# umr-lops/xsarsea

Hardware: AMD Instinct MI355X
Metric: Mpixels/s wind inversion (CMOD5.N, 20k x 20k sigma0) (higher is better)
Workload: dtype f64; 1 GPU; CMOD5.N mono-VV inversion (the metric's raster), 20000x20000 float32 sigma0/incidence + complex64 ancillary, default LUT 501x499x181 (90319 candidates/pixel), complex64 out, algo=pruned, sigma0 -> dB fused on the device; lines=20000, samples=20000, lines_rank0=20000, parallelism=row tiles x1

## Files before the change

profiles/band_vpipe_isa.py:

```python
#!/usr/bin/env python3
import collections
import os
import re
import subprocess
import sys
import tempfile

HERE = os.path.dirname(os.path.abspath(__file__))
sys.path.insert(0, HERE)
from stage1_isa_breakdown import CSRC, REPO, function_starts

KERNELS = [
    ("k_invert_band mono, table in LDS (the benchmark's)", "13k_invert_bandIffLb0ELb0ELi1ELb1EE"),
    ("k_invert_band mono, table in global memory", "13k_invert_bandIffLb0ELb0ELi1ELb0EE"),
    ("k_invert_band dual-pol, table in LDS", "13k_invert_bandIffLb1ELb0ELi1ELb1EE"),
    ("k_invert_band dual-pol, table in global memory", "13k_invert_bandIffLb1ELb0ELi1ELb0EE"),
    ("k_invert_band2 mono", "14k_invert_band2IffLb0EE"),
    ("k_invert_band2 dual-pol", "14k_invert_band2IffLb1EE"),
    ("k_invert_blocks mono", "15k_invert_blocksIffLb0EE"),
    ("k_invert_blocks dual-pol", "15k_invert_blocksIffLb1EE"),
]
HELPERS = {"vmin", "vmax", "vminf", "vmaxf", "dpp_d", "dpp_f", "seg_min_d", "wave_min_d", "rd_lane_d", "rd_lane_i", "mul24_sv", "wave_max_i",
           "ballot64", "byte_sum4", "ld", "to_db", "log10_fast"}
TAIL_FUNCS = {"wave_tail", "list_append", "mask_mark", "store_pixel", "angle_of_quotient", "hypot_glibc", "search_cr_scan", "search_cr_interval",
              "dsig_cr_at", "nearest_index_tail", "co_encode", "cr_encode", "store_opt"}
PASS_FUNCS = {"co_band_pass", "ld_co"}


def compile_asm(path):
    subprocess.check_call(["/opt/rocm/bin/hipcc", "--offload-arch=gfx950", "-O3", "-std=c++17", "-ffp-contract=off", "-I" + os.path.join(REPO, "include"),
                           "-I" + CSRC, "-DXSW_PAIR=0", "-gline-tables-only", "--cuda-device-only", "-S", os.path.join(CSRC, "xsw_invert_tu.hip"), "-o", path],
                          stderr=subprocess.DEVNULL)
    return open(path).read().split("\n")


def kind_of(op):
    if op.startswith(("global_", "flat_", "buffer_", "scratch_")):
        return "VMEM"
    if op.startswith("ds_"):
        return "LDS"
    if op.startswith(("s_load_", "s_buffer_load_")):
        return "SMEM"
    return "SALU" if op.startswith("s_") else "VALU"


def main():
    if len(sys.argv) > 1:
        text = open(sys.argv[1]).read().split("\n")
    else:
        with tempfile.TemporaryDirectory() as td:
            text = compile_asm(os.path.join(td, "tu.s"))
    files = {}
    for line in text:
        m = re.match(r'\s*\.file\s+(\d+)\s+"([^"]*)"\s+"([^"]*)"', line)
        if m:
            files[int(m.group(1))] = os.path.basename(m.group(3))
    headers = ("xsw_device.hpp", "xsw_band.hpp", "xsw_band2.hpp", "xsw_blocks.hpp", "xsw_codes.hpp")
    fstarts = {f: function_starts(os.path.join(CSRC, f)) for f in headers}
    band_src = open(os.path.join(CSRC, "xsw_band.hpp")).read().split("\n")
    l_passes = next(n for n, l in enumerate(band_src, 1) if "// ---- stage 2: band passes" in l)
    l_pickup = next(n for n, l in enumerate(band_src, 1) if "the workgroup's passes have settled every slot" in l)

    def phase_of(fname, line, prev):
        if fname not in fstarts:
# ... 89 lines not shown
```

xsarsea_amd/_build.py:

```python
import os
import shutil
import subprocess

HERE = os.path.dirname(os.path.abspath(__file__))
REPO = os.path.dirname(HERE)
CSRC = os.path.join(HERE, "csrc")
SRC = os.path.join(CSRC, "xsw.hip")
SRC_TU = os.path.join(CSRC, "xsw_invert_tu.hip")
SRC_GRAD = os.path.join(CSRC, "xsw_gradients.hip")
SRC_STREAKS = os.path.join(CSRC, "xsw_streaks.hip")
SRC_ANCILLARY = os.path.join(CSRC, "xsw_ancillary.hip")
SRC_CELLS = os.path.join(CSRC, "xsw_cells.hip")
SRC_CALIBRATE = os.path.join(CSRC, "xsw_calibrate.hip")
SRC_LANDMASK = os.path.join(CSRC, "xsw_landmask.hip")
DEPS = [os.path.join(CSRC, f) for f in sorted(os.listdir(CSRC)) if f.endswith((".hip", ".hpp"))] + [os.path.join(REPO, "include", "xsw.h")]
LIB = os.environ.get("XSW_LIB") or os.path.join(HERE, "libxsw.so")
OBJDIR = os.path.join(REPO, "build", "obj")
ARCH = "gfx950"


def hipcc():
    for cand in (shutil.which("hipcc"), "/opt/rocm/bin/hipcc"):
        if cand and os.path.exists(cand):
            return cand
    raise RuntimeError("hipcc not found: libxsw.so cannot be built")


def needs_build():
    if not os.path.exists(LIB):
        return True
    t = os.path.getmtime(LIB)
    return any(os.path.getmtime(d) > t for d in DEPS)


def build(force=False, verbose=False):
    if not force and not needs_build():
        return LIB
    cc = hipcc()
    extra = os.environ.get("XSW_EXTRA_FLAGS", "").split()
    tag = os.path.basename(LIB).replace(".", "_")
    os.makedirs(OBJDIR, exist_ok=True)
    common = [cc, f"--offload-arch={ARCH}", "-O3", "-std=c++17", "-ffp-contract=off", "-fPIC",
              "-I" + os.path.join(REPO, "include"), "-I" + CSRC] + extra
    jobs = [(SRC, os.path.join(OBJDIR, f"{tag}_main.o"), [])]
    jobs += [(SRC_TU, os.path.join(OBJDIR, f"{tag}_pair{k}.o"), [f"-DXSW_PAIR={k}"]) for k in range(4)]
    jobs += [(SRC_GRAD, os.path.join(OBJDIR, f"{tag}_gradients.o"), [])]
    jobs += [(SRC_STREAKS, os.path.join(OBJDIR, f"{tag}_streaks.o"), [])]
    jobs += [(SRC_ANCILLARY, os.path.join(OBJDIR, f"{tag}_ancillary.o"), [])]
    jobs += [(SRC_CELLS, os.path.join(OBJDIR, f"{tag}_cells.o"), [])]
    jobs += [(SRC_CALIBRATE, os.path.join(OBJDIR, f"{tag}_calibrate.o"), [])]
    jobs += [(SRC_LANDMASK, os.path.join(OBJDIR, f"{tag}_landmask.o"), [])]
    procs = []
    for src, obj, defs in jobs:
        cmd = common + defs + ["-c", src, "-o", obj]
        if verbose:
            print(" ".join(cmd))
        procs.append((cmd, subprocess.Popen(cmd)))
    failed = [cmd for cmd, p in procs if p.wait() != 0]
    if failed:
        raise subprocess.CalledProcessError(1, failed[0])
    link = [cc, f"--offload-arch={ARCH}", "-shared", "-fPIC", "-o", LIB] + [obj for _, obj, _ in jobs] + ["-Wl,-rpath,/opt/rocm/lib"]
    if verbose:
        print(" ".join(link))
    subprocess.check_call(link)
    return LIB


def _code_objects(lib, td):
    llvm = "/opt/rocm/lib/llvm/bin"
    fat = os.path.join(td, "fat.bin")
    subprocess.check_call([f"{llvm}/llvm-objcopy", "--dump-section", f".hip_fatbin={fat}", lib, os.path.join(td, "unused.so")])
    with open(fat, "rb") as f:
        blob = f.read()
    magic = b"__CLANG_OFFLOAD_BUNDLE__"
    starts = [m for m in range(len(blob)) if blob.startswith(magic, m)] if blob.count(magic) < 64 else []
    out = []
    for k, st in enumerate(starts):
        piece, co = os.path.join(td, f"bundle{k}.bin"), os.path.join(td, f"dev{k}.co")
# ... 81 lines not shown
```

xsarsea_amd/csrc/xsw.hip:

```cpp
#include <hip/hip_runtime.h>

#include <algorithm>
#include <atomic>
#include <chrono>
#include <limits>
#include <mutex>
#include <thread>
#include <cmath>
#include <cstdarg>
#include <cstdio>
#include <cstring>
#include <string>
#include <vector>

#include "xsw.h"
#include "xsw_device.hpp"
#include "xsw_misc.hpp"
#include "xsw_gmf.hpp"
#include "xsw_nesz.hpp"
#include "xsw_dsig.hpp"
#include "xsw_lutbuild.hpp"

using namespace xsw;

// ... 1 lines not shown

#define HIPCHK(c, expr)                                                                          \
    do {                                                                                         \
        hipError_t e_ = (expr);                                                                  \
        if (e_ != hipSuccess)                                                                    \
            return fail((c), e_ == hipErrorOutOfMemory ? XSW_ENOMEM : XSW_EHIP, "%s: %s (%s:%d)", \
                        #expr, hipGetErrorString(e_), __FILE__, __LINE__);                       \
    } while (0)

extern "C" int xsw_version(void) { return XSW_VERSION; }

extern "C" int xsw_device_count(void)
{
    int n = 0;
    if (hipGetDeviceCount(&n) != hipSuccess) return 0;
    return n;
}

extern "C" const char *xsw_last_error(const xsw_ctx *ctx) { return ctx ? ctx->err.c_str() : create_err().c_str(); }

extern "C" int xsw_ctx_create(int device, xsw_ctx **out)
{
    if (!out) return fail(nullptr, XSW_EINVAL, "ctx out pointer is NULL");
    *out = nullptr;
    int n = 0;
    hipError_t e = hipGetDeviceCount(&n);
    if (e != hipSuccess || n == 0)
        return fail(nullptr, XSW_EHIP, "no HIP device available (%s)", e == hipSuccess ? "count=0" : hipGetErrorString(e));
    if (device < 0 || device >= n) return fail(nullptr, XSW_EINVAL, "device %d out of range [0,%d)", device, n);
    xsw_ctx *c = new xsw_ctx;
    c->device = device;
    const int rc = [&]() -> int {
        HIPCHK(nullptr, hipSetDevice(device));
        HIPCHK(nullptr, hipStreamCreateWithFlags(&c->own_stream, hipStreamNonBlocking));
        c->stream = c->own_stream;
        HIPCHK(nullptr, hipMalloc((void **)&c->d_stats, 8 * sizeof(unsigned long long)));
        HIPCHK(nullptr, hipMemset(c->d_stats, 0, 8 * sizeof(unsigned long long)));
        return XSW_OK;
    }();
    if (rc != XSW_OK) {
        if (c->d_stats) (void)hipFree(c->d_stats);
        if (c->own_stream) (void)hipStreamDestroy(c->own_stream);
        delete c;
        return rc;
    }
    *out = c;
    return XSW_OK;
}

static void worker_release(xsw_ctx::Worker &w)
{
    if (w.s) (void)hipStreamSynchronize(w.s);
    (void)grow(w.pin, w.pin_cap, 0, nullptr, true);
    (void)grow(w.dev, w.dev_cap, 0);
}

extern "C" int xsw_ctx_destroy(xsw_ctx *c)
{
    if (!c) return XSW_OK;
    (void)hipSetDevice(c->device);
    (void)hipStreamSynchronize(c->stream);
    free_all(c->co_allocs);
    free_all(c->cr_allocs);
    if (c->d_stats) (void)hipFree(c->d_stats);
    (void)grow(c->d_ratio, c->ratio_cap, 0);
    (void)grow(c->lists.base, c->lists_bytes, 0);
// ... 1439 lines not shown
```

xsarsea_amd/csrc/xsw_band.hpp:

```cpp
#pragma once
#include "xsw_device.hpp"
#include "xsw_tilewalk.hpp"

namespace xsw {

#ifndef XSW_BAND_MAX
#define XSW_BAND_MAX 64
#endif
#ifndef XSW_BAND_RAY_D
#define XSW_BAND_RAY_D 2
#endif
#ifndef XSW_LONG_RUN_MAX
#define XSW_LONG_RUN_MAX 128
#endif
#ifndef XSW_LONG_RUN_MAX_CUT
#define XSW_LONG_RUN_MAX_CUT 64
#endif
#ifndef XSW_SWEEP_MAX
#define XSW_SWEEP_MAX 128
#endif
#ifndef XSW_B2_HARD_AREA
#define XSW_B2_HARD_AREA 256
#endif
#ifndef XSW_BAND_SEEDED
// ... 304 lines not shown
            atomicAdd(&A.stats[3], (unsigned long long)__popcll(done_cr));
        }
    }
    bool drop_b = false, drop_c = false;
    if (A.list_b) drop_b = A.rec_b ? (unresolved && to_b) : list_append(A.list_b_count, A.list_b, A.list_b_cap, unresolved && to_b, i, lane);
    if (A.list_c) drop_c = list_append(A.list_c_count, A.list_c, A.list_c_cap, unresolved && to_c && !to_b, i, lane);
    const bool for_c = A.list_c != nullptr && to_c && !to_b && !drop_c;
    const bool drop_g = list_append(A.list_count, A.list, A.list_cap, unresolved && !to_b && !for_c, i, lane);
    if (A.mask_g) {
        if (A.list_b) mask_mark(A.mask_b, drop_b, i, strip, A.samples, lane);
        mask_mark(A.mask_g, drop_g, i, strip, A.samples, lane);
    }
    if (in) {
        if (!unresolved) {
            Pixel Q;
            Q.flags = flags;
            Q.a_re = nan; Q.a_im = nan;
            if (A.anc) {
                typename Cx<T>::type z = ((const typename Cx<T>::type *)A.anc)[i];
                Q.a_re = (double)z.x;
                Q.a_im = (double)z.y;
            }
            store_pixel<TO, CR>(L, A, i, Q, my_flat, my_icr);
        }
    }
}

template <typename T, typename TO, bool CR, bool COUNT, int ROLE = 0, bool CSLDS = false>
__device__ __forceinline__ void band_wave(const DevTables &L, const KArgs &A, long long i, bool in, int lane, BandSlot *__restrict__ slots,
                                          int *__restrict__ res_ ,
                                          bool strip_walk = false ,
                                          long long strip = -1 ,
                                          BandPool *__restrict__ pool = nullptr ,
                                          double2 *cs_lds = nullptr )
{
    const double nan = __builtin_nan("");
    int flags, my_flat = -1, my_icr = -1;
    unsigned cand = 0;
    constexpr int NC = kBandClasses;
    constexpr bool POOLED = XSW_BAND_POOL && ROLE != 2;
    constexpr int WG = XSW_BAND_WG_WAVES, PK = POOLED ? 64 * WG : 64;
    const long long i_first = POOLED ? (long long)(((unsigned long long)(unsigned)__builtin_amdgcn_readfirstlane((int)((unsigned long long)i >> 32)) << 32) |
                                                   (unsigned)__builtin_amdgcn_readfirstlane((int)(unsigned)i)) : 0;
    int i_delta = POOLED ? (int)(i - i_first) : 0;
    int pos = -1, myc = NC, first[NC] = {}, ncls[NC] = {};
    auto settle_queues = [&]() {
#pragma unroll
        for (int c = 0; c + 1 < NC; ++c) {
            const int np = 64 / (2 << (c >> 1)), npn = 64 / (2 << ((c + 1) >> 1));
            const int rem = ncls[c] % np;
            const int added = (ncls[c + 1] + rem + npn - 1) / npn - (ncls[c + 1] + npn - 1) / npn;
            if (rem > 0 && added == 0) { ncls[c] -= rem; ncls[c + 1] += rem; first[c + 1] -= rem; }
        }
#pragma unroll
        for (int c = 0; c < NC; ++c) {
            first[c] = __builtin_amdgcn_readfirstlane(first[c]);
            ncls[c] = __builtin_amdgcn_readfirstlane(ncls[c]);
        }
    };
    bool skip = false;
    {
        Pixel P;
        load_pixel<T, false>(L, A, i, in, P);
        flags = P.flags;
        if (CR && A.s_cr) {
            const T x = ((const T *)A.s_cr)[i];
            const T dr = A.dsig_cr ? ((const T *)A.dsig_cr)[i] : (T)0;
// ... 151 lines not shown
                if (hm) {
                    unsigned at0 = 0;
                    if (lane == 0) at0 = atomicAdd(A1.list_b_count, (unsigned)__popcll(hm));
                    at0 = (unsigned)__builtin_amdgcn_readfirstlane((int)at0);
                    const unsigned at = at0 + __builtin_amdgcn_mbcnt_hi((unsigned)(hm >> 32), __builtin_amdgcn_mbcnt_lo((unsigned)hm, 0u));
                    if (to_rec && at < A1.list_b_cap) {
                        BandRec r;
                        r.s = P.s_co; r.ah = 0.5 * P.a_re; r.bh = 0.5 * P.b_eff; r.d = __double2float_ru(W.band_d);
                        r.inc_tail = P.i_inc | ((has_tail ? W.w_hi - w_hi_e : 0) << 16);
                        r.rows = W.w_lo | (w_hi_e << 16); r.ipn = W.ip_lo | (ncols_p << 16);
                        r.idx = (unsigned)i;
                        r.flags = (flags & ~F_TO_B) | (hard ? F_B2_HARD : 0);
                        ((BandRec *)A1.rec_b)[at] = r;
                        flags |= F_REC_DONE;
                    }
                }
            }
            if (eligb) {
#ifdef XSW_TIMING_STAGE1_ONLY
                b.res = 0;
#else
                b.res = -1;
#endif
                BandSlot &d = slots[pos];
                d.sn = b.sn; d.thr_lo = b.thr_lo; d.thr_hi = b.thr_hi; d.ah = b.ah; d.bh = b.bh;
                d.inc_bin = b.inc_bin; d.rows = b.rows; d.ipn = b.ipn; d.bin_hi = b.bin_hi;
                if constexpr (POOLED) d.res = b.res;
                else res_[pos] = b.res;
            }
        }
    }
    if constexpr (POOLED) slots[lane].pos = pos;
    else res_[PK + lane] = pos;
    const int wv = POOLED ? __builtin_amdgcn_readfirstlane((int)(threadIdx.x >> 6)) : 0;
    if constexpr (POOLED) {
        static_assert((WG & (WG - 1)) == 0, "passes are dealt to the waves modulo XSW_BAND_WG_WAVES");
        if (lane == 0) {
#pragma unroll
            for (int c = 0; c < NC; ++c) pool->cnt[c][wv] = (unsigned char)ncls[c];
        }
        double2 cs_in;
        const bool cs_mine = CSLDS && (int)threadIdx.x < L.n_phi;
        if constexpr (CSLDS) {
            static_assert(kBandCsCap <= 64 * WG, "one table entry per thread");
            if (cs_mine) cs_in = ((const double2 *)L.csphi)[threadIdx.x];
        }
        __syncthreads();
        int e = 0, base = 0;
#pragma unroll
        for (int c = 0; c < NC; ++c) {
            int n = 0, before = 0;
#pragma unroll
            for (int k = 0; k < WG / 4; ++k) {
                const unsigned x = (unsigned)__builtin_amdgcn_readfirstlane((int)((const unsigned *)pool->cnt[c])[k]);
                const int lo = wv - 4 * k;
                n += byte_sum4(x);
                before += byte_sum4(lo >= 4 ? x : lo <= 0 ? 0u : x & ((1u << (8 * lo)) - 1u));
            }
            e = myc == c ? base + before - first[c] : e;
            first[c] = base;
            ncls[c] = n;
            base += n;
        }
        settle_queues();
        if (pos >= 0) pool->map[pos + e] = (unsigned short)(wv * 64 + pos);
        if constexpr (CSLDS) {
            if (cs_mine) cs_lds[threadIdx.x] = cs_in;
        }
        __syncthreads();
    } else {
        __builtin_amdgcn_fence(__ATOMIC_RELEASE, "wavefront");
        __builtin_amdgcn_wave_barrier();
        __builtin_amdgcn_fence(__ATOMIC_ACQUIRE, "wavefront");
    }
#ifdef XSW_BAND_PASS_STATS
    unsigned long long pst[8] = {};
#endif
#ifndef XSW_TIMING_STAGE1_ONLY
    {
        int dealt = 0;
        auto run = [&](auto seg, auto kk, int c) {
            constexpr int S = decltype(seg)::value, K = decltype(kk)::value, np = 64 / S;
            if constexpr (POOLED) {
                const int npass = (ncls[c] + np - 1) / np;
                for (int p = (wv - dealt) & (WG - 1); p < npass; p += WG) {
                    co_band_pass<S, K, COUNT, true, CSLDS>(L, A.inv_dsig_co, lane, slots - 64 * wv, nullptr, first[c] + p * np, min(np, ncls[c] - p * np), cand,
                                                           pool->map, cs_lds);
#ifdef XSW_BAND_PASS_STATS
                    pst[c < 7 ? c : 7] += (1ULL << 32) + (unsigned long long)min(np, ncls[c] - p * np);
#endif
                }
                dealt += npass;
            } else {
                for (int p = 0; p < ncls[c]; p += np) {
                    co_band_pass<S, K, COUNT>(L, A.inv_dsig_co, lane, slots, res_, first[c] + p, min(np, ncls[c] - p), cand);
#ifdef XSW_BAND_PASS_STATS
                    pst[c < 7 ? c : 7] += (1ULL << 32) + (unsigned long long)min(np, ncls[c] - p);
#endif
                }
            }
        };
// ... 21 lines not shown
        __builtin_amdgcn_fence(__ATOMIC_RELEASE, "wavefront");
        __builtin_amdgcn_wave_barrier();
        __builtin_amdgcn_fence(__ATOMIC_ACQUIRE, "wavefront");
    }
#ifdef XSW_BAND_PASS_STATS
    if (A.stats && lane == 0) {
#pragma unroll
        for (int k = 0; k < 8; ++k)
            if (pst[k]) atomicAdd(&A.stats[k], pst[k]);
    }
#endif
    if constexpr (POOLED) {
        __asm__ volatile("" : "+v"(i_delta));
        i = i_first + i_delta;
        pos = slots[lane].pos;
        if (pos >= 0) my_flat = slots[pos].res;
    } else {
        pos = res_[PK + lane];
        if (pos >= 0) my_flat = res_[pos];
    }
    if (ROLE == 1 && (flags & F_REC_DONE) != 0) in = false;
    if (ROLE == 2 && strip_walk) {
        skip = skip || (flags & F_NEED_CO) == 0;
        in = in && !skip;
    }
    if constexpr (POOLED) {
        const KernArgs K = kernargs_again();
        wave_tail<T, TO, CR, COUNT>(*K.L, *K.A, i, in, lane, flags, my_flat, strip, cand);
    } else {
        wave_tail<T, TO, CR, COUNT>(L, A, i, in, lane, flags, my_flat, strip, cand);
    }
}

template <typename T, typename TO, bool CR, bool COUNT, int ROLE = 0, bool CSLDS = false>
__global__ __launch_bounds__(64 * XSW_BAND_WG_WAVES, CR ? XSW_BAND_WAVES_CR : XSW_BAND_WAVES) void k_invert_band(DevTables L, KArgs A)
{
    static_assert(!CSLDS || XSW_BAND_POOL, "the LDS copy of the direction table is published by the pooled queues' barriers");
    const int lane = threadIdx.x & 63, wv = threadIdx.x >> 6;
    __shared__ BandSlot slots[XSW_BAND_WG_WAVES][64];
#if XSW_BAND_POOL
    __shared__ BandPool pool;
    __shared__ double2 cs_lds[CSLDS ? kBandCsCap : 1];
#else
    __shared__ int res_[XSW_BAND_WG_WAVES][128];
#endif
    const long long strips_per_line = (A.samples + 63) >> 6;
    const long long band_groups = (A.lines + (XSW_BAND_WG_WAVES - 1)) / XSW_BAND_WG_WAVES;
    long long col_, group_;
    const bool tile_ = tile_walk(strips_per_line, band_groups, blockIdx.x & 7, blockIdx.y, blockIdx.x >> 3, col_, group_);
    const bool tile = __builtin_amdgcn_readfirstlane((int)tile_) != 0;
    unsigned col32 = (unsigned)__builtin_amdgcn_readfirstlane((int)col_), group32 = (unsigned)__builtin_amdgcn_readfirstlane((int)group_);
    __asm__ volatile("" : "+s"(col32), "+s"(group32));
    const long long col = col32, group = group32;
    const long long line = group * XSW_BAND_WG_WAVES + __builtin_amdgcn_readfirstlane(wv);
    const long long smp = col * 64 + lane;
#if XSW_BAND_POOL
    if (!tile) return;
    const bool live = line < A.lines;
    const bool in = live && smp < A.samples;
    const long long i = (live ? line : A.lines - 1) * A.samples + (smp < A.samples ? smp : A.samples - 1);
    band_wave<T, TO, CR, COUNT, ROLE, CSLDS>(L, A, i, in, lane, slots[wv], nullptr, false, line * strips_per_line + col, &pool, cs_lds);
#else
    if (!tile || line >= A.lines) return;
    const bool in = smp < A.samples;
    const long long i = line * A.samples + (in ? smp : A.samples - 1);
    band_wave<T, TO, CR, COUNT, ROLE>(L, A, i, in, lane, slots[wv], res_[wv], false, line * strips_per_line + col);
#endif
}

}
```

xsarsea_amd/csrc/xsw_device.hpp:

```cpp
#pragma once
#include <hip/hip_runtime.h>
#include <stdint.h>

#include <type_traits>

#include "xsw_codes.hpp"
#include "xsw_lutplan.hpp"
#include "xsw_tilewalk.hpp"

namespace xsw {

struct DevTables {
    const double *co;
    const double *coT;
    const double *inc, *w, *wh, *phi, *cphi, *sphi;
    const double *csphi;
    const float *csphi32;
    const float *co32;
    const float *wh32;
    double co_absmax;
    const double *out_dir;
    const double *abs_co;
    const double *dual_dir;
    const double *sol;
// ... 28 lines not shown
    const double *inv_cr_grid;
    int inc_cr_uniform;
    double inc_cr0, inv_inccrstep;
};

struct KArgs {
    const void *inc, *s_co, *s_cr, *dsig_cr, *anc;
    void *out_co, *out_cr;
    int *out_idx;
    unsigned *code_co, *code_cr;
    unsigned long long *stats;
    int stats_chain;
    unsigned *list;
    unsigned *list_count;
    unsigned list_cap;
    unsigned *list_b, *list_b_count;
    unsigned list_b_cap;
    void *rec_b;
    unsigned *list_c, *list_c_count;
    unsigned list_c_cap;
    unsigned long long *mask_g, *mask_b;
    int long_run;
    int tail_max;
    int area_max;
    int b2_crowd, area_crowd_max;
    int block_min;
    int arc_min, arc_crowd;
    int wide_min;
    int b2_refine_min;
    int b2_rows_max;
    long long n, lines, samples;
    double dsig_co, inv_dsig_co, dsig_cr_scalar;
    int is_db, dual_select;
};

enum : int { F_NEED_CO = 1, F_NEED_CR = 2, F_EARLY_NAN = 4, F_CO_FINITE = 8, F_CR_RAW_NAN = 16 ,
             F_CO_LOOSE = 32 ,
             F_REC_DONE = 256 ,
             F_B2_HARD = 512 ,
             F_B2_CROWD = 1024 ,
             F_TO_B = 64, F_TO_C = 128  };

__device__ __forceinline__ int rd_lane_i(int v, int l) { return __builtin_amdgcn_readlane(v, l); }
__device__ __forceinline__ double rd_lane_d(double v, int l)
{
    int lo = __builtin_amdgcn_readlane(__double2loint(v), l);
    int hi = __builtin_amdgcn_readlane(__double2hiint(v), l);
    return __hiloint2double(hi, lo);
}
__device__ __forceinline__ double vmin(double a, double b)
{
    double r;
    asm("v_min_f64 %0, %1, %2" : "=v"(r) : "v"(a), "v"(b));
    return r;
}
__device__ __forceinline__ double vmax(double a, double b)
{
    double r;
    asm("v_max_f64 %0, %1, %2" : "=v"(r) : "v"(a), "v"(b));
    return r;
}

__device__ __forceinline__ unsigned mul24_sv(unsigned uniform, unsigned v)
{
    unsigned r;
    asm("v_mul_u32_u24 %0, %1, %2" : "=v"(r) : "s"(uniform), "v"(v));
// ... 1257 lines not shown
```

xsarsea_amd/csrc/xsw_host.hpp:

```cpp
#pragma once
#include <hip/hip_runtime.h>

#include <climits>
#include <cstdarg>
#include <cstdint>
#include <cstdio>
#include <cstdlib>
#include <string>
#include <vector>

#include "xsw.h"
#include "xsw_device.hpp"
#include "xsw_plan.hpp"
#include "xsw_lutplan.hpp"

#ifndef XSW_ARENA_KEEP
#define XSW_ARENA_KEEP ((size_t)24 << 30)
#endif
struct xsw_ctx {
    int device = 0;
    hipStream_t own_stream = nullptr;
    hipStream_t stream = nullptr;
    xsw::DevTables T{};
    std::vector<void *> co_allocs, cr_allocs;
    bool have_co = false, have_cr = false;
    bool co_finite = false;
    unsigned long long *d_stats = nullptr;
    bool stats_on = false;
    bool stats_chain = false;
    bool timing_on = false;
    std::vector<hipEvent_t> timing_events;
    size_t lists_bytes = 0;
    WorkLists lists;
    double *d_ratio = nullptr;
    size_t ratio_cap = 0;
    void *nesz_scratch = nullptr;
    size_t nesz_cap = 0;
    struct Worker { hipStream_t s = nullptr; char *pin = nullptr; size_t pin_cap = 0; char *dev = nullptr; size_t dev_cap = 0; };
    std::vector<Worker> workers;
    int host_threads = 0;
    char *arena = nullptr;
    size_t arena_cap = 0;
    std::vector<void *> host_allocs;
    std::vector<double> h_sol, h_dual, h_wcr;
    std::vector<float> h_sol32;
    std::string err;
};


static inline void timing_mark(xsw_ctx *c)

{
    if (!c->timing_on) return;
// ... 76 lines not shown
    std::vector<void *> bufs;
    explicit CallTemps(hipStream_t s) : DevSeq{s, bufs} {}
    ~CallTemps() { if (!bufs.empty()) (void)finish(); }
    hipError_t finish()
    {
        const hipError_t e = hipStreamSynchronize(stream);
        free_all(bufs);
        return e;
    }
};

template <typename P>
static inline hipError_t grow(P *&ptr, size_t &cap, size_t need, const hipStream_t *wait_for = nullptr, bool pinned = false)
{
    hipError_t e = wait_for ? hipStreamSynchronize(*wait_for) : hipSuccess;
    if (e != hipSuccess) return e;
    if (ptr) (void)(pinned ? hipHostFree(ptr) : hipFree(ptr));
    ptr = nullptr;
    cap = 0;
    if (!need) return hipSuccess;
    e = pinned ? hipHostMalloc((void **)&ptr, need, hipHostMallocDefault) : hipMalloc((void **)&ptr, need);
    if (e == hipSuccess) cap = need;
    return e;
}

struct LaunchCtl {
    hipStream_t stream;
    bool timing;
    WorkLists lists;
};

static_assert(RouteFacts::PRUNED == XSW_ALGO_PRUNED && RouteFacts::EXHAUSTIVE == XSW_ALGO_EXHAUSTIVE && RouteFacts::EXACT == XSW_ALGO_EXACT &&
              RouteFacts::EXHAUSTIVE_F64 == XSW_ALGO_EXHAUSTIVE_F64, "RouteFacts::Algo (xsw_plan.hpp) is XSW_ALGO_*");
static inline RouteFacts route_facts(const xsw::DevTables &T, const xsw::KArgs &A, int algo, const LaunchCtl &lc)
{
    RouteFacts f;
    f.prunable = T.prunable; f.co_off32 = T.co_off32; f.band_mul24 = T.band_mul24; f.cr_monotone = T.cr_monotone; f.blk_span_ok = T.blk_span_ok;
    f.mono_rows = T.mono_rows; f.inv_rows = T.inv_rows; f.blk = T.blk; f.csphi32 = T.csphi32; f.tail_min = T.tail_min;
    f.n_w = T.n_w; f.n_phi = T.n_phi;
    f.lines = A.lines; f.samples = A.samples; f.n = A.n;
    f.algo = algo;
    f.s_co = A.s_co; f.s_cr = A.s_cr;
    f.mono = !A.s_cr && !A.out_cr && !A.code_cr;
    f.stats = A.stats; f.stats_chain = A.stats_chain;
    f.lists = lc.lists.base; f.mask_strips = lc.lists.mask_strips;
    return f;
}

static inline xsw::KArgs slice(const xsw::KArgs &A, const ChunkPlan::Chunk &ch, size_t es, size_t os)
{
    auto shift = [&](auto *p, size_t elem) -> decltype(p) { return p ? (decltype(p))((uintptr_t)p + ch.px0 * elem) : nullptr; };
    xsw::KArgs B = A;
    B.lines = ch.lines; B.samples = ch.samples; B.n = (long long)ch.npx;
    B.inc = shift(A.inc, es); B.s_co = shift(A.s_co, es); B.s_cr = shift(A.s_cr, es);
    B.dsig_cr = shift(A.dsig_cr, es); B.anc = shift(A.anc, es * 2);
    B.out_co = shift(A.out_co, os); B.out_cr = shift(A.out_cr, os);
    B.out_idx = shift(A.out_idx, 12);
    B.code_co = shift(A.code_co, 4); B.code_cr = shift(A.code_cr, 4);
    return B;
}

namespace xsw {
struct CrossArgs {
    const void *inc, *s_cr, *dsig_cr;
    const unsigned *code_co;
    unsigned *code_cr;
    void *out_cr;
    long long n;
    double dsig_cr_scalar;
// ... 87 lines not shown
```

xsarsea_amd/csrc/xsw_invert_tu.hip:

```cpp
#include <hip/hip_runtime.h>

#include <algorithm>
#include <string>
#include <type_traits>

#include "xsw_host.hpp"
#include "xsw_band.hpp"
#include "xsw_band2.hpp"
#include "xsw_blocks.hpp"
#include "xsw_exhaustive.hpp"
#include "xsw_cross.hpp"
#include "xsw_cost.hpp"
#include "xsw_uncertainty.hpp"
#include "xsw_forward.hpp"
#include "xsw_solve.hpp"
#include "xsw_dirsolve.hpp"
#include "xsw_joint.hpp"
#include "xsw_uncertainty_joint.hpp"

using namespace xsw;

template <typename F>
static void with_pol(bool dual, F &&f)
{
    if (dual) f(std::true_type{});
    else f(std::false_type{});
}

template <typename T, typename TO>
static int launch_invert(xsw_ctx *c, const KArgs &A_in, int algo, const LaunchCtl &lc, std::string &err)
{
    const RouteFacts f = route_facts(c->T, A_in, algo, lc);
    const ChainPlan p(route_knobs(), f, ChainWaves{XSW_BAND_WG_WAVES, XSW_BAND2_WAVES, XSW_BLOCKS_WAVES, XSW_BAND_POOL ? kBandCsCap : 0});
    if (p.route == ChainPlan::TOO_LARGE) return seterr(err, XSW_EINVAL, "raster too large for one launch");
    if (p.route == ChainPlan::EXHAUSTIVE)
        return launch_exhaustive<T, TO>(c->T, A_in, lc.stream, algo == XSW_ALGO_EXHAUSTIVE) == hipSuccess
                   ? XSW_OK : seterr(err, XSW_EHIP, "exhaustive launch failed: %s", hipGetErrorString(hipGetLastError()));
    KArgs A = A_in;
    A.block_min = p.block_min;
    if (p.route == ChainPlan::CHAIN) {
        KArgs B = A;
        const WorkLists &wl = lc.lists;
        B.list_count = wl.count(WorkLists::G); B.list = wl.entries(WorkLists::G); B.list_cap = wl.cap(WorkLists::G);
        if (p.band2) { B.list_b_count = wl.count(WorkLists::B); B.list_b = wl.entries(WorkLists::B); B.list_b_cap = wl.cap(WorkLists::B); }
        static_assert(sizeof(BandRec) == XSW_REC_BYTES, "XSW_REC_BYTES (xsw_plan.hpp) is sizeof(BandRec)");
        B.rec_b = p.records ? wl.records() : nullptr;
        if (p.blocks3) { B.list_c_count = wl.count(WorkLists::C); B.list_c = wl.entries(WorkLists::C); B.list_c_cap = wl.cap(WorkLists::C); }
        B.long_run = p.long_run; B.area_max = p.area_max; B.b2_crowd = p.b2_crowd; B.area_crowd_max = p.area_crowd_max;
        B.wide_min = p.wide_min; B.arc_min = p.arc_min; B.arc_crowd = p.arc_crowd; B.b2_refine_min = p.b2_refine_min;
        B.b2_rows_max = p.b2_rows_max; B.tail_max = p.tail_max;
        if (p.masks) {
            B.mask_g = wl.masks(); B.mask_b = wl.masks() + p.nstrips;
            if (hipMemsetAsync(wl.masks(), 0, 2 * p.nstrips * sizeof(unsigned long long), lc.stream) != hipSuccess) return seterr(err, XSW_EHIP, "strip-mask reset failed");
        }
        if (hipMemsetAsync(wl.count(WorkLists::G), 0, 3 * sizeof(unsigned), lc.stream) != hipSuccess) return seterr(err, XSW_EHIP, "work-list reset failed");
        const dim3 band_grid(p.band_grid_x, p.band_grid_y), band_block(64 * XSW_BAND_WG_WAVES);
        with_pol(!f.mono, [&](auto cr) {
            constexpr bool CR = decltype(cr)::value;
            if (lc.timing) timing_mark(c);
            auto band = [&](auto lds) {
                constexpr bool CSLDS = decltype(lds)::value;
                if (p.count_inst) hipLaunchKernelGGL((k_invert_band<T, TO, CR, true, 0, CSLDS>), band_grid, band_block, 0, lc.stream, c->T, B);
                else if (p.band2) hipLaunchKernelGGL((k_invert_band<T, TO, CR, false, 1, CSLDS>), band_grid, band_block, 0, lc.stream, c->T, B);
                else hipLaunchKernelGGL((k_invert_band<T, TO, CR, false, 0, CSLDS>), band_grid, band_block, 0, lc.stream, c->T, B);
            };
#if XSW_BAND_POOL
            if (p.cs_lds) band(std::true_type{});
            else
#endif
                band(std::false_type{});
            if (lc.timing) timing_mark(c);
#if defined(XSW_BAND_PASS_STATS) || defined(XSW_BAND_DETOUR_STATS)
            B.stats = nullptr;
#endif
            if (p.band2) hipLaunchKernelGGL((k_invert_band2<T, TO, CR>), dim3(p.band2_blocks), band_block, 0, lc.stream, c->T, B);
            if (lc.timing) timing_mark(c);
            if (p.blocks3) hipLaunchKernelGGL((k_invert_blocks<T, TO, CR>), dim3(p.blocks3_blocks), dim3(256), 0, lc.stream, c->T, B);
            if (lc.timing) timing_mark(c);
            hipLaunchKernelGGL((k_invert_list<T, TO, CR>), dim3(p.list_blocks), dim3(256), 0, lc.stream, c->T, B);
            if (lc.timing) timing_mark(c);
        });
    } else if (p.route == ChainPlan::ONE_PRUNED) {
        with_pol(!f.mono, [&](auto cr) {
            hipLaunchKernelGGL((k_invert<T, TO, 1, decltype(cr)::value>), dim3((unsigned)p.nblocks), dim3(256), 0, lc.stream, c->T, A);
        });
    } else {
        hipLaunchKernelGGL((k_invert<T, TO, 3>), dim3((unsigned)p.nblocks), dim3(256), 0, lc.stream, c->T, A);
    }
    const hipError_t e = hipGetLastError();
// ... 27 lines not shown
```

xsarsea_amd/csrc/xsw_plan.hpp:

```cpp
#pragma once
#include <algorithm>
#include <climits>
#include <cstddef>
#include <cstdlib>

#ifndef XSW_LIST_B_SHARE
#define XSW_LIST_B_SHARE 4
#endif
#ifndef XSW_LIST_C_SHARE
#define XSW_LIST_C_SHARE 4
#endif
#define XSW_LISTS_TOTAL (1 + XSW_LIST_B_SHARE + XSW_LIST_C_SHARE)
#define XSW_REC_BYTES 48

static inline size_t pad256(size_t b) { return (b + 255) & ~(size_t)255; }

struct WorkLists {
    enum List { G = 0, B = 1, C = 2 };
    unsigned *base = nullptr;
    size_t list_cap = 0;
    size_t mask_strips = 0;

    static size_t share(List l) { return l == G ? 1 : l == B ? XSW_LIST_B_SHARE : XSW_LIST_C_SHARE; }
    static size_t lists_bytes(size_t cap) { return pad256((XSW_LISTS_TOTAL * cap + 16) * sizeof(unsigned)); }
    size_t bytes() const
    {
        return lists_bytes(list_cap) + 2 * mask_strips * sizeof(unsigned long long) + (size_t)XSW_LIST_B_SHARE * list_cap * XSW_REC_BYTES;
    }

    unsigned *count(List l) const { return base + l; }
    unsigned *entries(List l) const { return base + 16 + (l == G ? 0 : l == B ? 1 : 1 + XSW_LIST_B_SHARE) * list_cap; }
    unsigned cap(List l) const { return (unsigned)std::min<size_t>(share(l) * list_cap, 0xfffffff0u); }
    unsigned long long *masks() const { return (unsigned long long *)((char *)base + lists_bytes(list_cap)); }
    void *records() const { return masks() + 2 * mask_strips; }
};

static inline size_t strips_for(long long n, long long lines) { return (size_t)(n / 64 + std::max<long long>(lines, n / 4096) + 64); }

static inline size_t context_list_cap(long long n, long long test_cap)
{
    return ((size_t)(test_cap ? test_cap : std::max<long long>(n / 8, 1 << 16)) + 1) & ~(size_t)1;
}
static inline size_t worker_list_cap(size_t max_px) { return std::max<size_t>(max_px / 8, 1 << 14) & ~(size_t)1; }

struct ChunkPlan {
    long long lines, samples;
    long long lines_per_chunk, nmain, tail_px, nchunks;
    size_t max_px;

    struct Chunk {
        size_t px0, npx;
        long long lines, samples;
    };

    ChunkPlan(long long lines_in, long long samples_in, long long cap_px, long long tile_rows, bool recut_flat)
        : lines(lines_in), samples(samples_in), tail_px(0)
    {
        const long long n = lines * samples;
        if (recut_flat && lines < 16 && n >= (1LL << 16)) { samples = 4096; lines = n / samples; tail_px = n - lines * samples; }
        lines_per_chunk = lines;
        if (cap_px > 0) {
            const long long target_px = std::min<long long>(cap_px, std::max<long long>(1LL << 16, n / 16));
            lines_per_chunk = samples > 0 ? (target_px + samples - 1) / samples : lines;
// ... 59 lines not shown
#endif
#ifndef XSW_B2_REFINE_MIN
#define XSW_B2_REFINE_MIN 16
#endif
#ifndef XSW_B2_ROWS_MAX
#define XSW_B2_ROWS_MAX 4096
#endif
#ifndef XSW_TAIL_SWEEP
#define XSW_TAIL_SWEEP 256
#endif
#ifndef XSW_BLOCK_MIN
#define XSW_BLOCK_MIN 1024
#endif

static inline long long env_int(const char *name, long long dflt, long long lo = LLONG_MIN, long long hi = LLONG_MAX)
{
    const char *v = getenv(name);
    return v ? std::min(std::max(atoll(v), lo), hi) : dflt;
}
static inline bool env_flag(const char *name) { return getenv(name) != nullptr; }

struct RouteKnobs {
    int block_min = XSW_BLOCK_MIN;
    bool no_band = false;
    int long_run = XSW_LONG_RUN_DEFAULT;
    bool no_records = false;
    bool no_blocks_kernel = false;
    int b2_area = XSW_B2_AREA, b2_crowd = XSW_B2_CROWD , b2_wide = XSW_B2_WIDE;
    int arc_min = XSW_ARC_MIN, arc_crowd = XSW_ARC_CROWD;
    int b2_refine_min = XSW_B2_REFINE_MIN, b2_rows_max = XSW_B2_ROWS_MAX, tail_sweep = XSW_TAIL_SWEEP;
    bool no_strip_masks = false;
    long long list_cap_test = 0;
    bool fail_list_alloc = false;

    static RouteKnobs from_env()
    {
        RouteKnobs k;
        k.block_min = (int)env_int("XSW_BLOCK_MIN", XSW_BLOCK_MIN, 0);
        k.no_band = env_flag("XSW_NO_BAND");
        k.long_run = (int)env_int("XSW_LONG_RUN", XSW_LONG_RUN_DEFAULT, 0);
        k.no_records = env_flag("XSW_NO_RECORDS");
        k.no_blocks_kernel = env_flag("XSW_NO_BLOCKS_KERNEL");
        k.b2_area = (int)env_int("XSW_B2_AREA", XSW_B2_AREA, 1);
        k.b2_crowd = (int)env_int("XSW_B2_CROWD", XSW_B2_CROWD, 1);
        k.b2_wide = (int)env_int("XSW_B2_WIDE", XSW_B2_WIDE, 0);
        k.arc_min = (int)env_int("XSW_ARC_MIN", XSW_ARC_MIN);
        k.arc_crowd = (int)env_int("XSW_ARC_CROWD", XSW_ARC_CROWD, 1);
        k.b2_refine_min = (int)env_int("XSW_B2_REFINE_MIN", XSW_B2_REFINE_MIN, 0);
        k.b2_rows_max = (int)env_int("XSW_B2_ROWS_MAX", XSW_B2_ROWS_MAX, 1);
        k.tail_sweep = (int)env_int("XSW_TAIL_SWEEP", XSW_TAIL_SWEEP, 0, 30000);
        k.no_strip_masks = env_flag("XSW_NO_STRIP_MASKS");
        k.list_cap_test = env_int("XSW_LIST_CAP_TEST", 0, 16);
        k.fail_list_alloc = env_flag("XSW_FAIL_LIST_ALLOC");
        return k;
    }
};

struct RouteFacts {
    enum Algo { PRUNED = 1, EXHAUSTIVE = 2, EXACT = 3, EXHAUSTIVE_F64 = 4 };
    bool prunable, co_off32, band_mul24, cr_monotone, blk_span_ok;
    bool mono_rows, inv_rows, blk, csphi32, tail_min;
    int n_w, n_phi;
    long long lines, samples, n;
    int algo;
    bool s_co, s_cr;
    bool mono;
    bool stats, stats_chain;
    bool lists;
    size_t mask_strips;
};

struct ChainWaves {
    int band_wg, band2, blocks;
    int band_cs_cap = 0;
};

struct ChainPlan {
    enum Route { EXHAUSTIVE, CHAIN, ONE_PRUNED, ONE_EXACT, TOO_LARGE };
    enum Limit { NONE, NBLOCKS, BAND_GROUPS, BAND_COLS };
    Route route;
    Limit limit = NONE;
    long long nblocks;
    int block_min;
    bool count_inst = false;
    bool band2 = false;
    bool records = false;
    bool blocks3 = false;
    bool cs_lds = false;
    bool masks = false;
    size_t nstrips = 0;
    int long_run = 0, area_max = 0, b2_crowd = 0, area_crowd_max = 0, wide_min = 0, arc_min = 0, arc_crowd = 0, b2_refine_min = 0,
        b2_rows_max = 0, tail_max = 0;
    unsigned band_grid_x = 0, band_grid_y = 0, band2_blocks = 0, blocks3_blocks = 0, list_blocks = 0;

    ChainPlan(const RouteKnobs &k, const RouteFacts &f, const ChainWaves &w) : block_min(k.block_min)
    {
        const long long strips_per_line = (f.samples + 63) / 64, line_groups = (f.lines + 3) / 4;
        nblocks = 8 * ((strips_per_line + 7) / 8) * line_groups;
        if (nblocks > 0x7fffffffLL) { route = TOO_LARGE; limit = NBLOCKS; return; }
        if (f.algo == RouteFacts::EXHAUSTIVE || f.algo == RouteFacts::EXHAUSTIVE_F64) { route = EXHAUSTIVE; return; }
        if (!(f.algo == RouteFacts::PRUNED && !k.no_band && f.lists && f.s_co && f.prunable && f.mono_rows && f.inv_rows && f.co_off32 &&
              f.band_mul24 && (!f.s_cr || f.cr_monotone) && f.n < (1LL << 32))) {
            route = f.algo == RouteFacts::PRUNED ? ONE_PRUNED : ONE_EXACT;
            return;
        }
        const long long cols_per_xcd = (strips_per_line + 7) / 8;
        const long long band_groups = (f.lines + w.band_wg - 1) / w.band_wg;
        if (8 * band_groups > 0x7fffffffLL) { route = TOO_LARGE; limit = BAND_GROUPS; return; }
        if (cols_per_xcd > 65535) { route = TOO_LARGE; limit = BAND_COLS; return; }
        route = CHAIN;
        count_inst = f.stats && !f.stats_chain;
        band2 = k.long_run > 0 && !count_inst;
        records = band2 && !k.no_records;
        cs_lds = f.n_phi >= 1 && f.n_phi <= w.band_cs_cap;
        blocks3 = f.blk && f.blk_span_ok && !k.no_blocks_kernel && f.n_w < 32768 && f.n_phi < 32768;
        long_run = k.long_run;
        area_max = f.blk ? k.b2_area : 0x7fffffff;
        b2_crowd = k.b2_crowd;
        area_crowd_max = 1 << 20;
        wide_min = k.b2_wide > 0 ? k.b2_wide : 0x7fffffff;
        arc_min = (k.arc_min > 0 && f.csphi32) ? k.arc_min : 0x7fffffff;
        arc_crowd = k.arc_crowd;
        b2_refine_min = k.b2_refine_min;
        b2_rows_max = k.b2_rows_max;
        tail_max = (band2 && f.tail_min) ? k.tail_sweep : 0;
        nstrips = (size_t)(strips_per_line * f.lines);
        masks = nstrips <= f.mask_strips && !k.no_strip_masks;
        band_grid_x = (unsigned)(8 * band_groups);
        band_grid_y = (unsigned)cols_per_xcd;
        band2_blocks = (unsigned)std::min<long long>(nblocks, 256 * w.band2);
        blocks3_blocks = (unsigned)std::min<long long>(nblocks, 256 * w.blocks);
        list_blocks = (unsigned)std::min<long long>(nblocks, 256 * 8);
    }
};
```

xsarsea_amd/csrc/xsw_tilewalk.hpp:

```cpp
#pragma once

#if defined(__HIPCC__) || defined(__CUDACC__)
#define XSW_TILEWALK_HD __host__ __device__
#else
#define XSW_TILEWALK_HD
#endif

namespace xsw {

XSW_TILEWALK_HD inline bool tile_walk(long long strips, long long lg, long long xcd, long long y, long long g, long long &col,
                                      long long &group)
{
    const long long base = strips >> 3, rem = strips & 7;
    col = xcd * base + y;
    group = g;
    if (y < base) return true;
    if (y > base || rem == 0) return false;
    const long long left = rem * lg, q = (left + 7) >> 3;
    long long t = xcd * q + g;
    if (g >= q || t >= left) return false;
    col = 8 * base;
    while (t >= lg) {
        t -= lg;
        ++col;
    }
    group = t;
    return true;
}

XSW_TILEWALK_HD inline bool tile_walk_linear(long long strips, long long lg, long long b, long long &col, long long &group)
{
    const long long j = b >> 3;
    return tile_walk(strips, lg, b & 7, j / lg, j % lg, col, group);
}

}
```

Baseline: 11710 Mpixels/s.

## Make band kernel persistent with per-XCD ticket queues and hoisted direction table

Replaces the one-workgroup-per-tile grid of the pooled band kernel with a resident grid sized from the CU count. Each workgroup pulls runs of tiles from per-XCD queues through atomic tickets and steals from other XCD queues once its own is drained. The LDS copy of the direction table is loaded once per workgroup instead of once per tile. The TU build also disables machine LICM to limit register pressure in the now-looping kernel. This is meant to cut launch and tail imbalance and per-workgroup setup cost, at the price of atomics, extra barriers and a more complex loop with re-read kernel arguments.

```diff
diff --git a/profiles/band_vpipe_isa.py b/profiles/band_vpipe_isa.py
--- a/profiles/band_vpipe_isa.py
+++ b/profiles/band_vpipe_isa.py
@@ -27,9 +27,18 @@
 PASS_FUNCS = {"co_band_pass", "ld_co"}
 
 
+def tu_flags():
+    import importlib.util
+    spec = importlib.util.spec_from_file_location("xsw_build", os.path.join(REPO, "xsarsea_amd", "_build.py"))
+    mod = importlib.util.module_from_spec(spec)
+    spec.loader.exec_module(mod)
+    return list(mod.TU_FLAGS)
+
+
 def compile_asm(path):
     subprocess.check_call(["/opt/rocm/bin/hipcc", "--offload-arch=gfx950", "-O3", "-std=c++17", "-ffp-contract=off", "-I" + os.path.join(REPO, "include"),
-                           "-I" + CSRC, "-DXSW_PAIR=0", "-gline-tables-only", "--cuda-device-only", "-S", os.path.join(CSRC, "xsw_invert_tu.hip"), "-o", path],
+                           "-I" + CSRC, "-DXSW_PAIR=0"] + tu_flags() + [
+                           "-gline-tables-only", "--cuda-device-only", "-S", os.path.join(CSRC, "xsw_invert_tu.hip"), "-o", path],
                           stderr=subprocess.DEVNULL)
     return open(path).read().split("\n")
 
diff --git a/xsarsea_amd/_build.py b/xsarsea_amd/_build.py
--- a/xsarsea_amd/_build.py
+++ b/xsarsea_amd/_build.py
@@ -17,6 +17,7 @@
 LIB = os.environ.get("XSW_LIB") or os.path.join(HERE, "libxsw.so")
 OBJDIR = os.path.join(REPO, "build", "obj")
 ARCH = "gfx950"
+TU_FLAGS = ["-mllvm", "-disable-machine-licm"]
 
 
 def hipcc():
@@ -43,7 +44,7 @@
     common = [cc, f"--offload-arch={ARCH}", "-O3", "-std=c++17", "-ffp-contract=off", "-fPIC",
               "-I" + os.path.join(REPO, "include"), "-I" + CSRC] + extra
     jobs = [(SRC, os.path.join(OBJDIR, f"{tag}_main.o"), [])]
-    jobs += [(SRC_TU, os.path.join(OBJDIR, f"{tag}_pair{k}.o"), [f"-DXSW_PAIR={k}"]) for k in range(4)]
+    jobs += [(SRC_TU, os.path.join(OBJDIR, f"{tag}_pair{k}.o"), [f"-DXSW_PAIR={k}"] + TU_FLAGS) for k in range(4)]
     jobs += [(SRC_GRAD, os.path.join(OBJDIR, f"{tag}_gradients.o"), [])]
     jobs += [(SRC_STREAKS, os.path.join(OBJDIR, f"{tag}_streaks.o"), [])]
     jobs += [(SRC_ANCILLARY, os.path.join(OBJDIR, f"{tag}_ancillary.o"), [])]
diff --git a/xsarsea_amd/csrc/xsw.hip b/xsarsea_amd/csrc/xsw.hip
--- a/xsarsea_amd/csrc/xsw.hip
+++ b/xsarsea_amd/csrc/xsw.hip
@@ -57,6 +57,7 @@
     c->device = device;
     const int rc = [&]() -> int {
         HIPCHK(nullptr, hipSetDevice(device));
+        HIPCHK(nullptr, hipDeviceGetAttribute(&c->cus, hipDeviceAttributeMultiprocessorCount, device));
         HIPCHK(nullptr, hipStreamCreateWithFlags(&c->own_stream, hipStreamNonBlocking));
         c->stream = c->own_stream;
         HIPCHK(nullptr, hipMalloc((void **)&c->d_stats, 8 * sizeof(unsigned long long)));
diff --git a/xsarsea_amd/csrc/xsw_band.hpp b/xsarsea_amd/csrc/xsw_band.hpp
--- a/xsarsea_amd/csrc/xsw_band.hpp
+++ b/xsarsea_amd/csrc/xsw_band.hpp
@@ -360,7 +360,9 @@
                                           bool strip_walk = false ,
                                           long long strip = -1 ,
                                           BandPool *__restrict__ pool = nullptr ,
-                                          double2 *cs_lds = nullptr )
+                                          const double2 *cs_lds = nullptr ,
+                                          unsigned *tk_count = nullptr, unsigned *tk_lds = nullptr ,
+                                          int wave = 0 )
 {
     const double nan = __builtin_nan("");
     int flags, my_flat = -1, my_icr = -1;
@@ -578,19 +580,16 @@
     }
     if constexpr (POOLED) slots[lane].pos = pos;
     else res_[PK + lane] = pos;
-    const int wv = POOLED ? __builtin_amdgcn_readfirstlane((int)(threadIdx.x >> 6)) : 0;
+    const int wv = POOLED ? __builtin_amdgcn_readfirstlane(wave) : 0;
     if constexpr (POOLED) {
         static_assert((WG & (WG - 1)) == 0, "passes are dealt to the waves modulo XSW_BAND_WG_WAVES");
         if (lane == 0) {
 #pragma unroll
             for (int c = 0; c < NC; ++c) pool->cnt[c][wv] = (unsigned char)ncls[c];
         }
-        double2 cs_in;
-        const bool cs_mine = CSLDS && (int)threadIdx.x < L.n_phi;
-        if constexpr (CSLDS) {
-            static_assert(kBandCsCap <= 64 * WG, "one table entry per thread");
-            if (cs_mine) cs_in = ((const double2 *)L.csphi)[threadIdx.x];
-        }
+        unsigned tk_in = 0;
+        const bool tk_mine = tk_count != nullptr && wv == 0 && lane == 0;
+        if (tk_mine) tk_in = atomicAdd(tk_count, 1u);
         __syncthreads();
         int e = 0, base = 0;
 #pragma unroll
@@ -610,9 +609,7 @@
         }
         settle_queues();
         if (pos >= 0) pool->map[pos + e] = (unsigned short)(wv * 64 + pos);
-        if constexpr (CSLDS) {
-            if (cs_mine) cs_lds[threadIdx.x] = cs_in;
-        }
+        if (tk_mine) *tk_lds = tk_in;
         __syncthreads();
     } else {
         __builtin_amdgcn_fence(__ATOMIC_RELEASE, "wavefront");
@@ -700,18 +697,73 @@
     }
 }
 
+#ifndef XSW_BAND_RUN
+#define XSW_BAND_RUN 4
+#endif
+static_assert(XSW_BAND_RUN == 1 || XSW_BAND_RUN == 2 || XSW_BAND_RUN == 4 || XSW_BAND_RUN == 8, "queue positions per ticket");
+
 template <typename T, typename TO, bool CR, bool COUNT, int ROLE = 0, bool CSLDS = false>
 __global__ __launch_bounds__(64 * XSW_BAND_WG_WAVES, CR ? XSW_BAND_WAVES_CR : XSW_BAND_WAVES) void k_invert_band(DevTables L, KArgs A)
 {
     static_assert(!CSLDS || XSW_BAND_POOL, "the LDS copy of the direction table is published by the pooled queues' barriers");
-    const int lane = threadIdx.x & 63, wv = threadIdx.x >> 6;
     __shared__ BandSlot slots[XSW_BAND_WG_WAVES][64];
 #if XSW_BAND_POOL
     __shared__ BandPool pool;
     __shared__ double2 cs_lds[CSLDS ? kBandCsCap : 1];
+    __shared__ unsigned tk_lds;
+    if constexpr (CSLDS) {
+        static_assert(kBandCsCap <= 64 * XSW_BAND_WG_WAVES, "one table entry per thread");
+        if ((int)threadIdx.x < L.n_phi) cs_lds[threadIdx.x] = ((const double2 *)L.csphi)[threadIdx.x];
+    }
+    const unsigned lanes = gridDim.x >> 3;
+    unsigned q = blockIdx.x & 7, seen = 0;
+    unsigned p = (blockIdx.x >> 3) << A.band_run_shift, pe = p;
+#pragma unroll 1
+    for (;;) {
+        unsigned tid = threadIdx.x;
+        __asm__ volatile("" : "+v"(tid));
+        const int lane = (int)(tid & 63), wv = (int)(tid >> 6);
+        const KernArgs K = kernargs_again();
+        const long long samples = K.A->samples, lines = K.A->lines;
+        const unsigned gs = K.A->band_run_shift, G = 1u << gs;
+        const long long strips_per_line = (samples + 63) >> 6;
+        const long long band_groups = (lines + (XSW_BAND_WG_WAVES - 1)) / XSW_BAND_WG_WAVES;
+        if (p == pe) {
+            const unsigned n = (unsigned)tile_queue_len(strips_per_line, band_groups, q);
+            if (p >= n) {
+                if (++seen == 8) break;
+                q = (q + 1) & 7;
+                __syncthreads();
+                if (tid == 0) tk_lds = atomicAdd(K.A->band_tickets + q, 1u);
+                __syncthreads();
+                p = (lanes + (unsigned)__builtin_amdgcn_readfirstlane((int)*(volatile unsigned *)&tk_lds)) << gs;
+                pe = p;
+                continue;
+            }
+            pe = min(p + G, n);
+        }
+        long long col_, group_;
+        (void)tile_queue_at(strips_per_line, band_groups, K.A->lg_magic, q, p, col_, group_);
+        unsigned col32 = (unsigned)__builtin_amdgcn_readfirstlane((int)col_), group32 = (unsigned)__builtin_amdgcn_readfirstlane((int)group_);
+        __asm__ volatile("" : "+s"(col32), "+s"(group32));
+        const long long col = col32, group = group32;
+        const long long line = group * XSW_BAND_WG_WAVES + __builtin_amdgcn_readfirstlane(wv);
+        const long long smp = col * 64 + lane;
+        const bool live = line < lines;
+        const bool in = live && smp < samples;
+        const long long i = (live ? line : lines - 1) * samples + (smp < samples ? smp : samples - 1);
+        const bool draw = (p & (G - 1)) == 0;
+        band_wave<T, TO, CR, COUNT, ROLE, CSLDS>(*K.L, *K.A, i, in, lane, slots[wv], nullptr, false, line * strips_per_line + col, &pool, cs_lds,
+                                                 draw ? K.A->band_tickets + q : nullptr, &tk_lds, wv);
+        if (++p == pe) {
+            const unsigned gs_again = kernargs_again().A->band_run_shift;
+            p = (lanes + (unsigned)__builtin_amdgcn_readfirstlane((int)*(volatile unsigned *)&tk_lds)) << gs_again;
+            pe = p;
+        }
+    }
 #else
+    const int lane = threadIdx.x & 63, wv = threadIdx.x >> 6;
     __shared__ int res_[XSW_BAND_WG_WAVES][128];
-#endif
     const long long strips_per_line = (A.samples + 63) >> 6;
     const long long band_groups = (A.lines + (XSW_BAND_WG_WAVES - 1)) / XSW_BAND_WG_WAVES;
     long long col_, group_;
@@ -722,13 +774,6 @@
     const long long col = col32, group = group32;
     const long long line = group * XSW_BAND_WG_WAVES + __builtin_amdgcn_readfirstlane(wv);
     const long long smp = col * 64 + lane;
-#if XSW_BAND_POOL
-    if (!tile) return;
-    const bool live = line < A.lines;
-    const bool in = live && smp < A.samples;
-    const long long i = (live ? line : A.lines - 1) * A.samples + (smp < A.samples ? smp : A.samples - 1);
-    band_wave<T, TO, CR, COUNT, ROLE, CSLDS>(L, A, i, in, lane, slots[wv], nullptr, false, line * strips_per_line + col, &pool, cs_lds);
-#else
     if (!tile || line >= A.lines) return;
     const bool in = smp < A.samples;
     const long long i = line * A.samples + (in ? smp : A.samples - 1);
diff --git a/xsarsea_amd/csrc/xsw_device.hpp b/xsarsea_amd/csrc/xsw_device.hpp
--- a/xsarsea_amd/csrc/xsw_device.hpp
+++ b/xsarsea_amd/csrc/xsw_device.hpp
@@ -84,6 +84,9 @@
     long long n, lines, samples;
     double dsig_co, inv_dsig_co, dsig_cr_scalar;
     int is_db, dual_select;
+    unsigned *band_tickets;
+    unsigned lg_magic;
+    unsigned band_run_shift;
 };
 
 enum : int { F_NEED_CO = 1, F_NEED_CR = 2, F_EARLY_NAN = 4, F_CO_FINITE = 8, F_CR_RAW_NAN = 16 ,
diff --git a/xsarsea_amd/csrc/xsw_host.hpp b/xsarsea_amd/csrc/xsw_host.hpp
--- a/xsarsea_amd/csrc/xsw_host.hpp
+++ b/xsarsea_amd/csrc/xsw_host.hpp
@@ -19,6 +19,7 @@
 #endif
 struct xsw_ctx {
     int device = 0;
+    int cus = 0;
     hipStream_t own_stream = nullptr;
     hipStream_t stream = nullptr;
     xsw::DevTables T{};
@@ -161,9 +162,10 @@
 
 static_assert(RouteFacts::PRUNED == XSW_ALGO_PRUNED && RouteFacts::EXHAUSTIVE == XSW_ALGO_EXHAUSTIVE && RouteFacts::EXACT == XSW_ALGO_EXACT &&
               RouteFacts::EXHAUSTIVE_F64 == XSW_ALGO_EXHAUSTIVE_F64, "RouteFacts::Algo (xsw_plan.hpp) is XSW_ALGO_*");
-static inline RouteFacts route_facts(const xsw::DevTables &T, const xsw::KArgs &A, int algo, const LaunchCtl &lc)
+static inline RouteFacts route_facts(const xsw::DevTables &T, const xsw::KArgs &A, int algo, const LaunchCtl &lc, int cus)
 {
     RouteFacts f;
+    f.cus = cus;
     f.prunable = T.prunable; f.co_off32 = T.co_off32; f.band_mul24 = T.band_mul24; f.cr_monotone = T.cr_monotone; f.blk_span_ok = T.blk_span_ok;
     f.mono_rows = T.mono_rows; f.inv_rows = T.inv_rows; f.blk = T.blk; f.csphi32 = T.csphi32; f.tail_min = T.tail_min;
     f.n_w = T.n_w; f.n_phi = T.n_phi;
diff --git a/xsarsea_amd/csrc/xsw_invert_tu.hip b/xsarsea_amd/csrc/xsw_invert_tu.hip
--- a/xsarsea_amd/csrc/xsw_invert_tu.hip
+++ b/xsarsea_amd/csrc/xsw_invert_tu.hip
@@ -30,8 +30,8 @@
 template <typename T, typename TO>
 static int launch_invert(xsw_ctx *c, const KArgs &A_in, int algo, const LaunchCtl &lc, std::string &err)
 {
-    const RouteFacts f = route_facts(c->T, A_in, algo, lc);
-    const ChainPlan p(route_knobs(), f, ChainWaves{XSW_BAND_WG_WAVES, XSW_BAND2_WAVES, XSW_BLOCKS_WAVES, XSW_BAND_POOL ? kBandCsCap : 0});
+    const RouteFacts f = route_facts(c->T, A_in, algo, lc, c->cus);
+    const ChainPlan p(route_knobs(), f, ChainWaves{XSW_BAND_WG_WAVES, XSW_BAND2_WAVES, XSW_BLOCKS_WAVES, XSW_BAND_POOL ? kBandCsCap : 0, XSW_BAND_WAVES, XSW_BAND_WAVES_CR, XSW_BAND_RUN});
     if (p.route == ChainPlan::TOO_LARGE) return seterr(err, XSW_EINVAL, "raster too large for one launch");
     if (p.route == ChainPlan::EXHAUSTIVE)
         return launch_exhaustive<T, TO>(c->T, A_in, lc.stream, algo == XSW_ALGO_EXHAUSTIVE) == hipSuccess
@@ -49,12 +49,13 @@
         B.long_run = p.long_run; B.area_max = p.area_max; B.b2_crowd = p.b2_crowd; B.area_crowd_max = p.area_crowd_max;
         B.wide_min = p.wide_min; B.arc_min = p.arc_min; B.arc_crowd = p.arc_crowd; B.b2_refine_min = p.b2_refine_min;
         B.b2_rows_max = p.b2_rows_max; B.tail_max = p.tail_max;
+        B.band_tickets = wl.tickets(); B.lg_magic = p.lg_magic; B.band_run_shift = p.band_run_shift;
         if (p.masks) {
             B.mask_g = wl.masks(); B.mask_b = wl.masks() + p.nstrips;
             if (hipMemsetAsync(wl.masks(), 0, 2 * p.nstrips * sizeof(unsigned long long), lc.stream) != hipSuccess) return seterr(err, XSW_EHIP, "strip-mask reset failed");
         }
-        if (hipMemsetAsync(wl.count(WorkLists::G), 0, 3 * sizeof(unsigned), lc.stream) != hipSuccess) return seterr(err, XSW_EHIP, "work-list reset failed");
-        const dim3 band_grid(p.band_grid_x, p.band_grid_y), band_block(64 * XSW_BAND_WG_WAVES);
+        if (hipMemsetAsync(wl.count(WorkLists::G), 0, WorkLists::reset_words * sizeof(unsigned), lc.stream) != hipSuccess) return seterr(err, XSW_EHIP, "work-list reset failed");
+        const dim3 band_grid = XSW_BAND_POOL ? dim3(p.band_resident) : dim3(p.band_grid_x, p.band_grid_y), band_block(64 * XSW_BAND_WG_WAVES);
         with_pol(!f.mono, [&](auto cr) {
             constexpr bool CR = decltype(cr)::value;
             if (lc.timing) timing_mark(c);
diff --git a/xsarsea_amd/csrc/xsw_plan.hpp b/xsarsea_amd/csrc/xsw_plan.hpp
--- a/xsarsea_amd/csrc/xsw_plan.hpp
+++ b/xsarsea_amd/csrc/xsw_plan.hpp
@@ -4,6 +4,8 @@
 #include <cstddef>
 #include <cstdlib>
 
+#include "xsw_tilewalk.hpp"
+
 #ifndef XSW_LIST_B_SHARE
 #define XSW_LIST_B_SHARE 4
 #endif
@@ -29,6 +31,8 @@
     }
 
     unsigned *count(List l) const { return base + l; }
+    unsigned *tickets() const { return base + 8; }
+    static constexpr size_t reset_words = 16;
     unsigned *entries(List l) const { return base + 16 + (l == G ? 0 : l == B ? 1 : 1 + XSW_LIST_B_SHARE) * list_cap; }
     unsigned cap(List l) const { return (unsigned)std::min<size_t>(share(l) * list_cap, 0xfffffff0u); }
     unsigned long long *masks() const { return (unsigned long long *)((char *)base + lists_bytes(list_cap)); }
@@ -154,6 +158,7 @@
     bool no_strip_masks = false;
     long long list_cap_test = 0;
     bool fail_list_alloc = false;
+    long long band_resident_wgs = 0;
 
     static RouteKnobs from_env()
     {
@@ -174,6 +179,7 @@
         k.no_strip_masks = env_flag("XSW_NO_STRIP_MASKS");
         k.list_cap_test = env_int("XSW_LIST_CAP_TEST", 0, 16);
         k.fail_list_alloc = env_flag("XSW_FAIL_LIST_ALLOC");
+        k.band_resident_wgs = env_int("XSW_BAND_RESIDENT_WGS", 0, 0, 1 << 20);
         return k;
     }
 };
@@ -190,11 +196,14 @@
     bool stats, stats_chain;
     bool lists;
     size_t mask_strips;
+    int cus = 0;
 };
 
 struct ChainWaves {
     int band_wg, band2, blocks;
     int band_cs_cap = 0;
+    int band_wgs = 8, band_wgs_cr = 7;
+    int band_run = 4;
 };
 
 struct ChainPlan {
@@ -214,6 +223,7 @@
     int long_run = 0, area_max = 0, b2_crowd = 0, area_crowd_max = 0, wide_min = 0, arc_min = 0, arc_crowd = 0, b2_refine_min = 0,
         b2_rows_max = 0, tail_max = 0;
     unsigned band_grid_x = 0, band_grid_y = 0, band2_blocks = 0, blocks3_blocks = 0, list_blocks = 0;
+    unsigned band_resident = 0, lg_magic = 0, band_run_shift = 0;
 
     ChainPlan(const RouteKnobs &k, const RouteFacts &f, const ChainWaves &w) : block_min(k.block_min)
     {
@@ -250,6 +260,15 @@
         masks = nstrips <= f.mask_strips && !k.no_strip_masks;
         band_grid_x = (unsigned)(8 * band_groups);
         band_grid_y = (unsigned)cols_per_xcd;
+        {
+            const long long cus = f.cus > 0 ? f.cus : 256, per_cu = f.mono ? w.band_wgs : w.band_wgs_cr;
+            long long lanes = std::max<long long>(cus / 8, 1) * std::max<long long>(per_cu, 1);
+            lanes = std::min(lanes, std::max<long long>(strips_per_line * band_groups / 8, 1));
+            if (k.band_resident_wgs > 0) lanes = std::min(lanes, std::max<long long>(k.band_resident_wgs / 8, 1));
+            band_resident = (unsigned)(8 * lanes);
+            while ((2LL << band_run_shift) <= w.band_run && (2LL << band_run_shift) * band_resident <= strips_per_line * band_groups) ++band_run_shift;
+            lg_magic = xsw::tile_queue_magic(band_groups);
+        }
         band2_blocks = (unsigned)std::min<long long>(nblocks, 256 * w.band2);
         blocks3_blocks = (unsigned)std::min<long long>(nblocks, 256 * w.blocks);
         list_blocks = (unsigned)std::min<long long>(nblocks, 256 * 8);
diff --git a/xsarsea_amd/csrc/xsw_tilewalk.hpp b/xsarsea_amd/csrc/xsw_tilewalk.hpp
--- a/xsarsea_amd/csrc/xsw_tilewalk.hpp
+++ b/xsarsea_amd/csrc/xsw_tilewalk.hpp
@@ -34,4 +34,41 @@
     return tile_walk(strips, lg, b & 7, j / lg, j % lg, col, group);
 }
 
+XSW_TILEWALK_HD inline unsigned tile_queue_magic(long long lg)
+{
+    const unsigned long long m = (1ULL << 32) / (unsigned long long)(lg > 0 ? lg : 1);
+    return m > 0xffffffffULL ? 0xffffffffu : (unsigned)m;
 }
+
+XSW_TILEWALK_HD inline long long tile_queue_len(long long strips, long long lg, long long xcd)
+{
+    const long long base = strips >> 3, left = (strips & 7) * lg, q = (left + 7) >> 3;
+    long long mine = left - xcd * q;
+    mine = mine < 0 ? 0 : mine > q ? q : mine;
+    return base * lg + mine;
+}
+
+XSW_TILEWALK_HD inline bool tile_queue_at(long long strips, long long lg, unsigned lg_magic, long long xcd, long long p, long long &col, long long &group)
+{
+    const long long base = strips >> 3, own = base * lg;
+    if (p >= own) return tile_walk(strips, lg, xcd, base, p - own, col, group);
+    long long y = (long long)(((unsigned long long)(unsigned)p * lg_magic) >> 32);
+    long long g = p - y * lg;
+    if (g >= lg) {
+        g -= lg;
+        ++y;
+    }
+    col = xcd * base + y;
+    group = g;
+    return true;
+}
+
+XSW_TILEWALK_HD inline long long tile_ticket(long long strips, long long lg, long long xcd, long long t, long long G, long long &first)
+{
+    const long long n = tile_queue_len(strips, lg, xcd);
+    first = t * G;
+    const long long left = n - first;
+    return left <= 0 ? 0 : left < G ? left : G;
+}
+
+}
```

Result: faster. 12380 Mpixels/s (median of 6 runs) (+5.7%).
